# TrevorS/voxtral-mini-realtime-rs

Hardware: AMD Instinct MI355X
Metric: decode_tok_per_s (higher is better)
Workload: dtype f32

## Files before the change

voxtral-mini-realtime-rs_amd/csrc/vox_kernels.hip:

```cpp
#include "vox_kernels.h"

#include <hip/hip_fp16.h>

#include <unistd.h>

#include <algorithm>
#include <atomic>
#include <cstdio>
#include <cstdlib>
#include <cstring>
#include <string>
#include <mutex>
#include <unordered_map>

namespace vox {

static int g_tl_next = -1, g_tl_slots = 0;
#ifdef VOX_TIMELINE
__device__ unsigned long long* g_tl_buf = nullptr;
__device__ int g_tl_waves = 0;
__device__ __forceinline__ void tl_stamp(int slot, int wave_global, int k) {
    if (slot >= 0 && (wave_global & 3) == 0 && (threadIdx.x & 63) == 0 && g_tl_buf && wave_global < g_tl_waves)
        g_tl_buf[((size_t)slot * g_tl_waves + wave_global) * 4 + k] = wall_clock64();
}
// ... 483 lines not shown
    const int P = passes_for(p.w.K, R);
#define VOX_RP(R_, P_) if (R == R_ && P == P_) return gemv_dispatch_pe<P_, R_>(p, ny, pro, epi, s)
    VOX_RP(1, 1); VOX_RP(1, 2); VOX_RP(1, 3); VOX_RP(1, 5);
    VOX_RP(2, 1); VOX_RP(2, 2); VOX_RP(2, 3); VOX_RP(2, 4); VOX_RP(2, 5); VOX_RP(2, 9);
    VOX_RP(4, 1); VOX_RP(4, 2); VOX_RP(4, 6);
#undef VOX_RP
    return hipErrorInvalidValue;
}

const char* q4_gemv_kernel_name(int K, int pro, int epi, int R) {
    static thread_local char buf[96];
    snprintf(buf, sizeof buf, "q4_gemv_kernel<P=%d,R=%d,PRO=%d,EPI=%d,NWV=%d>", passes_for(K, R), R, pro, epi, gemv_fat_shape(K, R) ? q4_gemv_nwv(K, epi) : 4);
    return buf;
}

__device__ __forceinline__ float dot8_bf16(const uint4 w, const float4 xa, const float4 xb) {
    float s0 = __uint_as_float(w.x << 16) * xa.x, s1 = __uint_as_float(w.x & 0xFFFF0000u) * xa.y;
    s0 = fmaf(__uint_as_float(w.y << 16), xa.z, s0); s1 = fmaf(__uint_as_float(w.y & 0xFFFF0000u), xa.w, s1);
    s0 = fmaf(__uint_as_float(w.z << 16), xb.x, s0); s1 = fmaf(__uint_as_float(w.z & 0xFFFF0000u), xb.y, s1);
    s0 = fmaf(__uint_as_float(w.w << 16), xb.z, s0); s1 = fmaf(__uint_as_float(w.w & 0xFFFF0000u), xb.w, s1);
    return s0 + s1;
}

__device__ __forceinline__ float dot8_f32(const uint4 we, const uint4 wo, const float4 xa, const float4 xb) {
    float s0 = __uint_as_float(we.x) * xa.x, s1 = __uint_as_float(we.y) * xa.y;
    s0 = fmaf(__uint_as_float(we.z), xa.z, s0); s1 = fmaf(__uint_as_float(we.w), xa.w, s1);
    s0 = fmaf(__uint_as_float(wo.x), xb.x, s0); s1 = fmaf(__uint_as_float(wo.y), xb.y, s1);
    s0 = fmaf(__uint_as_float(wo.z), xb.z, s0); s1 = fmaf(__uint_as_float(wo.w), xb.w, s1);
    return s0 + s1;
}
template <int PRO, int EPI, int F32W = 0>
__global__ __launch_bounds__(256) VOX_NO_PK_F32 void dense_gemv_kernel(const GemvParams p) {
    constexpr int NX = 10, R = 2;
    extern __shared__ __attribute__((aligned(16))) float smem[];
    const int K = p.w.K, N = p.w.N, nc = K >> 3;
    float4* xe = reinterpret_cast<float4*>(smem);
    float4* xo = xe + nc;
    float* red = smem + K;
    const int tid = threadIdx.x, lane = tid & 63, wave = tid >> 6, y = blockIdx.y;
    const float* __restrict__ xg = p.x + (size_t)y * p.x_stride;
    const int npieces = K >> 2;
    float4 xp[NX];
    float ss = 0.f;
#pragma unroll
    for (int i = 0; i < NX; i++) {
        const int pc = tid + 256 * i;
        xp[i] = reinterpret_cast<const float4*>(xg)[min(pc, npieces - 1)];
        if (PRO != PRO_NONE && pc < npieces) ss += (xp[i].x * xp[i].x + xp[i].y * xp[i].y) + (xp[i].z * xp[i].z + xp[i].w * xp[i].w);
    }
    float rms = 1.0f;
    if (PRO != PRO_NONE) {
        ss = wave_sum(ss);
        if (lane == 0) red[wave] = ss;
        __syncthreads();
        rms = 1.0f / sqrtf(((red[0] + red[1]) + (red[2] + red[3])) / (float)K + p.eps);
    }
#pragma unroll
    for (int i = 0; i < NX; i++) {
        const int pc = tid + 256 * i;
        if (pc < npieces) {
            float4 v = xp[i];
            if (PRO != PRO_NONE) {
                const float4 gm = reinterpret_cast<const float4*>(p.gamma)[pc];
                v.x = (v.x * rms) * gm.x; v.y = (v.y * rms) * gm.y; v.z = (v.z * rms) * gm.z; v.w = (v.w * rms) * gm.w;
                if (PRO == PRO_RMS_MUL) {
                    const float4 m = reinterpret_cast<const float4*>(p.mul)[pc];
                    v.x *= m.x; v.y *= m.y; v.z *= m.z; v.w *= m.w;
                }
            }
            if (pc & 1) xo[pc >> 1] = v; else xe[pc >> 1] = v;
        }
    }
    __syncthreads();
    int best_i = 0x7fffffff; float best = -INFINITY;
    const int pos = (EPI == EPI_ROPE_KV) ? (p.pos_ptr ? *p.pos_ptr : 0) + p.pos_off : 0;
    const int n_groups = N / R, n_waves = gridDim.x * 4;
    for (int g = blockIdx.x * 4 + wave; g < n_groups; g += n_waves) {
        const int row0 = g * R;
        const uint4* w0 = (F32W ? p.w.qt : p.w.qs) + (size_t)row0 * nc * (F32W ? 2 : 1);
        const uint4* w1 = w0 + nc * (F32W ? 2 : 1);
        float acc[R] = {0.f, 0.f};
        for (int c0 = 0; c0 < nc; c0 += 128) {
            const int ca = c0 + lane, cb = ca + 64, cca = min(ca, nc - 1), ccb = min(cb, nc - 1);
            const float4 xea = xe[cca], xoa = xo[cca], xeb = xe[ccb], xob = xo[ccb];
            const float ma = ca < nc ? 1.0f : 0.0f, mb = cb < nc ? 1.0f : 0.0f;
            if (F32W) {
                const uint4 a0e = ld_nt_u4(w0 + 2 * cca), a0o = ld_nt_u4(w0 + 2 * cca + 1), a1e = ld_nt_u4(w0 + 2 * ccb), a1o = ld_nt_u4(w0 + 2 * ccb + 1);
                const uint4 b0e = ld_nt_u4(w1 + 2 * cca), b0o = ld_nt_u4(w1 + 2 * cca + 1), b1e = ld_nt_u4(w1 + 2 * ccb), b1o = ld_nt_u4(w1 + 2 * ccb + 1);
                acc[0] += ma * dot8_f32(a0e, a0o, xea, xoa) + mb * dot8_f32(a1e, a1o, xeb, xob);
                acc[1] += ma * dot8_f32(b0e, b0o, xea, xoa) + mb * dot8_f32(b1e, b1o, xeb, xob);
            } else {
                const uint4 a0 = ld_nt_u4(w0 + cca), a1 = ld_nt_u4(w0 + ccb), b0 = ld_nt_u4(w1 + cca), b1 = ld_nt_u4(w1 + ccb);
                acc[0] += ma * dot8_bf16(a0, xea, xoa) + mb * dot8_bf16(a1, xeb, xob);
                acc[1] += ma * dot8_bf16(b0, xea, xoa) + mb * dot8_bf16(b1, xeb, xob);
            }
        }
        acc[0] = wave_sum(acc[0]); acc[1] = wave_sum(acc[1]);
        if (EPI == EPI_STORE || EPI == EPI_RESID || EPI == EPI_GELU) {
#pragma unroll
            for (int r = 0; r < R; r++) {
                const int n = row0 + r;
                if (lane == r) {
                    float v = acc[r];
                    if (p.bias) v += p.bias[n];
                    if (EPI == EPI_RESID) v = v + p.resid[(size_t)y * p.resid_stride + n];
                    if (EPI == EPI_GELU) v = gelu_f(v);
                    p.out[(size_t)y * p.out_stride + n] = v;
                }
            }
        } else if (EPI == EPI_SWIGLU) {
            if (lane == 0) p.out[(size_t)y * p.out_stride + (row0 >> 1)] = silu_f(acc[0]) * acc[1];
        } else if (EPI == EPI_ROPE_KV) {
            const int hd = p.hd, half = hd >> 1, n = row0;
            if (lane == 0) {
                const float a = acc[0], b = acc[1];
                if (n < p.n_q + p.n_k) {
                    const int dd = n % hd;
                    const float c = p.rope_cos[(size_t)pos * half + (dd >> 1)], sn = p.rope_sin[(size_t)pos * half + (dd >> 1)];
                    const float ra = a * c - b * sn, rb = a * sn + b * c;
                    if (n < p.n_q) { p.out[n] = ra; p.out[n + 1] = rb; }
                    else {
                        const int kn = n - p.n_q, kh = kn / hd;
                        float* dst = p.kcache + (size_t)kh * p.cache_head_stride + (size_t)pos * hd + dd;
                        dst[0] = ra; dst[1] = rb;
                    }
                } else {
                    const int vn = n - p.n_q - p.n_k, vh = vn / hd, dd = vn % hd;
                    float* dst = p.vcache + (size_t)vh * p.cache_head_stride + (size_t)pos * hd + dd;
                    dst[0] = a; dst[1] = b;
                }
            }
        } else if (EPI == EPI_ARGMAX) {
#pragma unroll
            for (int r = 0; r < R; r++) {
                const int n = row0 + r;
                if (p.out && lane == r) p.out[(size_t)y * p.out_stride + n] = acc[r];
                argmax_take(best, best_i, acc[r], n);
            }
        }
    }
    if (EPI == EPI_ARGMAX) {
        if (lane == 0) { red[4 + wave] = best; reinterpret_cast<int*>(red)[8 + wave] = best_i; }
        __syncthreads();
        if (tid == 0) {
            float bv = red[4]; int bidx = reinterpret_cast<int*>(red)[8];
            for (int wv = 1; wv < 4; wv++) argmax_take(bv, bidx, red[4 + wv], reinterpret_cast<int*>(red)[8 + wv]);
            p.part_val[(size_t)y * gridDim.x + blockIdx.x] = bv;
            p.part_idx[(size_t)y * gridDim.x + blockIdx.x] = bidx;
        }
    }
}

int dense_gemv_grid(int N) { const int wgs = (N / 2 + 3) / 4; return wgs > 2048 ? 2048 : (wgs < 1 ? 1 : wgs); }

template <int PRO, int EPI>
static hipError_t dense_launch_t(const GemvParams& p, int ny, hipStream_t s) {
    const size_t lds = (size_t)(p.w.K + 16) * sizeof(float);
    gemm_form_note(GEMM_FORM_DENSE_GEMV);
    if (p.w.fmt == WFMT_F32) dense_gemv_kernel<PRO, EPI, 1><<<dim3(dense_gemv_grid(p.w.N), ny), dim3(256), lds, s>>>(p);
    else dense_gemv_kernel<PRO, EPI, 0><<<dim3(dense_gemv_grid(p.w.N), ny), dim3(256), lds, s>>>(p);
    return hipGetLastError();
}
static hipError_t launch_dense_gemv(const GemvParams& p, int ny, int pro, int epi, hipStream_t s) {
    if (p.w.K % 32 || p.w.K > 10240 || p.w.N % 2) return hipErrorInvalidValue;
    if ((pro == PRO_RMS_MUL || pro == PRO_RMS_MUL_SUM) && p.mul == nullptr) return hipErrorInvalidValue;
    if (pro == PRO_RMS_MUL_SUM) return hipErrorInvalidValue;
#define VOX_CASE(P_, E_) if (pro == P_ && epi == E_) return dense_launch_t<P_, E_>(p, ny, s)
    VOX_CASE(PRO_NONE, EPI_STORE); VOX_CASE(PRO_NONE, EPI_RESID); VOX_CASE(PRO_NONE, EPI_GELU); VOX_CASE(PRO_NONE, EPI_SWIGLU);
    VOX_CASE(PRO_RMS, EPI_STORE); VOX_CASE(PRO_RMS, EPI_ARGMAX); VOX_CASE(PRO_RMS, EPI_SWIGLU); VOX_CASE(PRO_RMS_MUL, EPI_SWIGLU);
    VOX_CASE(PRO_RMS, EPI_ROPE_KV);
#undef VOX_CASE
    return hipErrorInvalidValue;
}

typedef __attribute__((__vector_size__(8 * sizeof(__bf16)))) __bf16 bf16x8;
typedef __attribute__((__vector_size__(4 * sizeof(float)))) float f32x4;

__device__ __forceinline__ uint32_t bf16_rne_bits(float x) {
    const uint32_t u = __float_as_uint(x);
    return (u + 0x7FFFu + ((u >> 16) & 1u)) >> 16;
}
typedef __bf16 bf16x2_t __attribute__((ext_vector_type(2)));
typedef float f32x2_t __attribute__((ext_vector_type(2)));
__device__ __forceinline__ uint32_t cvt_pk_bf16(float a, float b) {
    const f32x2_t v = {a, b};
    union { bf16x2_t b; uint32_t u; } c; c.b = __builtin_convertvector(v, bf16x2_t); return c.u;
}
__device__ __forceinline__ void split_pair(float a, float b, uint32_t& hi, uint32_t& lo) {
    hi = cvt_pk_bf16(a, b);
    lo = cvt_pk_bf16(a - __uint_as_float(hi << 16), b - __uint_as_float(hi & 0xFFFF0000u));
}
__device__ __forceinline__ void split_bf16x8(const float4 a, const float4 b, uint4& hi, uint4& lo) {
    split_pair(a.x, a.y, hi.x, lo.x); split_pair(a.z, a.w, hi.y, lo.y);
    split_pair(b.x, b.y, hi.z, lo.z); split_pair(b.z, b.w, hi.w, lo.w);
}
__device__ __forceinline__ uint32_t pack_bf16_exact(float a, float b) {
    return (__float_as_uint(a) >> 16) | (__float_as_uint(b) & 0xFFFF0000u);
}
__device__ __forceinline__ uint4 q4_dword_to_bf16x8(uint32_t w) {
    const uint32_t lo = w & 0x0F0F0F0Fu, hi = (w >> 4) & 0x0F0F0F0Fu;
    uint4 o;
    o.x = pack_bf16_exact(ub0(lo) - 8.0f, ub1(lo) - 8.0f);
    o.y = pack_bf16_exact(ub2(lo) - 8.0f, ub3(lo) - 8.0f);
    o.z = pack_bf16_exact(ub0(hi) - 8.0f, ub1(hi) - 8.0f);
    o.w = pack_bf16_exact(ub2(hi) - 8.0f, ub3(hi) - 8.0f);
    return o;
}
__device__ __forceinline__ bf16x8 as_bf16x8(uint4 v) {
    union { uint4 u; bf16x8 b; } c; c.u = v; return c.b;
}

__device__ __forceinline__ uint4 q4_dword_to_bf16x8_biased(uint32_t w) {
    const uint32_t lo = w & 0x0F0F0F0Fu, hi = (w >> 4) & 0x0F0F0F0Fu, c = 0x43434343u;
    return make_uint4(__builtin_amdgcn_perm(lo, c, 0x00060004u), __builtin_amdgcn_perm(hi, c, 0x00060004u),
                      __builtin_amdgcn_perm(lo, c, 0x00070005u), __builtin_amdgcn_perm(hi, c, 0x00070005u));
}

__device__ __forceinline__ void xf_store4(uint16_t* __restrict__ xf, int K, int row, int k, float4 v) {
    const int q = k >> 7, j = (k >> 5) & 3, e = k & 31, half = e >> 4, g = (e & 15) >> 2;
    const size_t base = ((size_t)((q * 4 + j) * 64 + g * 16 + row)) * 8 + 2 * half;
    const size_t plane = (size_t)(K >> 7) * 256 * 8;
    uint32_t hi, lo;
    split_pair(v.x, v.z, hi, lo); *reinterpret_cast<uint32_t*>(xf + base) = hi; *reinterpret_cast<uint32_t*>(xf + plane + base) = lo;
    split_pair(v.y, v.w, hi, lo); *reinterpret_cast<uint32_t*>(xf + base + 4) = hi; *reinterpret_cast<uint32_t*>(xf + plane + base + 4) = lo;
}

template <int EPI, int FMT>
__global__ __launch_bounds__(256) __attribute__((amdgpu_waves_per_eu(2))) void q4_gemm_k32_kernel(const GemmParams p) {
    __shared__ __attribute__((aligned(16))) uint4 lds[2][2][256];
    const int K = p.w.K, nb = p.w.nb, N = p.w.N, M = p.M;
    (void)K;
    const int tid = threadIdx.x, lane = tid & 63, wave = tid >> 6;
    const int m0 = blockIdx.y * 64, n0 = blockIdx.x * 64;
    const int sm = tid >> 2, sg = tid & 3;
    const bool srow_ok = (m0 + sm) < M;
    const float* xrow = p.x + (size_t)(srow_ok ? (m0 + sm) : 0) * p.x_stride;
    const int slot = ((sm >> 4) * 4 + sg) * 16 + (sm & 15);
    const int wn = n0 + wave * 16 + (lane & 15), wg = lane >> 4;
    const bool wrow_ok = wn < N;
    const uint32_t* wq = reinterpret_cast<const uint32_t*>(p.w.qs) + (size_t)(wrow_ok ? wn : 0) * nb * 4 + wg;
    const uint16_t* ws = FMT == WFMT_Q4_0 ? p.w.sc + (size_t)(wrow_ok ? wn : 0) * nb : nullptr;
    const uint4* wd16 = p.w.qs + (size_t)(wrow_ok ? wn : 0) * nb * 4 + wg;
    const int xoff_a = FMT == WFMT_Q4_0 ? 4 * sg : 8 * sg, xoff_b = FMT == WFMT_Q4_0 ? 16 + 4 * sg : 8 * sg + 4;

    f32x4 acc[4];
#pragma unroll
    for (int i = 0; i < 4; i++) acc[i] = (f32x4){0.f, 0.f, 0.f, 0.f};

#define VOX_GLOAD(B_)                                                                              \
    xa = *reinterpret_cast<const float4*>(xrow + 32 * (B_) + xoff_a);        \
    xb = *reinterpret_cast<const float4*>(xrow + 32 * (B_) + xoff_b);                                               \
    if (FMT == WFMT_Q4_0) { wd = wq[(size_t)(B_) * 4]; wsc = ws[(B_)]; }    \
    else { wdv = wd16[(size_t)(B_) * 4]; }
#define VOX_STAGE(BUF_)                                                                            \
    { uint4 hi_, lo_; split_bf16x8(xa, xb, hi_, lo_); lds[(BUF_)][0][slot] = hi_; lds[(BUF_)][1][slot] = lo_; }
    float4 xa, xb; uint32_t wd = 0; uint16_t wsc = 0; uint4 wdv = make_uint4(0, 0, 0, 0);
    VOX_GLOAD(0)
    VOX_STAGE(0)
    uint32_t cur_wd = wd; uint16_t cur_sc = wsc; uint4 cur_wdv = wdv;
    { const int b1 = min(1, nb - 1); VOX_GLOAD(b1) }
    __syncthreads();
    for (int b = 0; b < nb; b++) {
        const int buf = b & 1;
        const float4 sxa = xa, sxb = xb; const uint32_t swd = wd; const uint16_t ssc = wsc; const uint4 swdv = wdv;
        { const int b2 = min(b + 2, nb - 1); VOX_GLOAD(b2) }
        const bf16x8 bw = as_bf16x8(FMT == WFMT_Q4_0 ? q4_dword_to_bf16x8(cur_wd) : cur_wdv);
        const float d = FMT == WFMT_Q4_0 ? f16_bits_to_f32(cur_sc) : 1.0f;
#pragma unroll
        for (int mt = 0; mt < 4; mt++) {
            const bf16x8 ah = as_bf16x8(lds[buf][0][mt * 64 + lane]);
            const bf16x8 al = as_bf16x8(lds[buf][1][mt * 64 + lane]);
            f32x4 t = __builtin_amdgcn_mfma_f32_16x16x32_bf16(ah, bw, (f32x4){0.f, 0.f, 0.f, 0.f}, 0, 0, 0);
            t = __builtin_amdgcn_mfma_f32_16x16x32_bf16(al, bw, t, 0, 0, 0);
            acc[mt][0] = fmaf(d, t[0], acc[mt][0]); acc[mt][1] = fmaf(d, t[1], acc[mt][1]);
            acc[mt][2] = fmaf(d, t[2], acc[mt][2]); acc[mt][3] = fmaf(d, t[3], acc[mt][3]);
        }
        if (b + 1 < nb) {
            uint4 hi_, lo_; split_bf16x8(sxa, sxb, hi_, lo_); lds[buf ^ 1][0][slot] = hi_; lds[buf ^ 1][1][slot] = lo_;
            cur_wd = swd; cur_sc = ssc; cur_wdv = swdv;
        }
        __syncthreads();
    }
#undef VOX_GLOAD
#undef VOX_STAGE
    const float bias = (p.bias && wrow_ok) ? p.bias[wn] : 0.f;
#pragma unroll
    for (int mt = 0; mt < 4; mt++)
#pragma unroll
        for (int r = 0; r < 4; r++) {
            const int m = m0 + mt * 16 + 4 * (lane >> 4) + r;
            float v = acc[mt][r] + bias;
            if (EPI == EPI_SWIGLU) {
                const float other = dpp_mov<0xB1>(v);
                if (m < M && wrow_ok && !(wn & 1)) p.out[(size_t)m * p.out_stride + (wn >> 1)] = silu_f(v) * other;
            } else if (m < M && wrow_ok) {
                if (EPI == EPI_RESID) v = v + p.resid[(size_t)m * p.resid_stride + wn];
                if (EPI == EPI_GELU) v = gelu_f(v);
                p.out[(size_t)m * p.out_stride + wn] = v;
            }
        }
}

template <int MT, int NT, int EPI, int FMT, int TB = 0>
__global__ __launch_bounds__(256) __attribute__((amdgpu_waves_per_eu(2))) void q4_gemm_kernel(const GemmParams p) {
    extern __shared__ __attribute__((aligned(16))) uint4 glds[];
    constexpr int PLANE = 4 * MT * 64, BUF = 2 * PLANE;
    const int nb = p.w.nb, N = p.w.N, M = p.M, nq = nb >> 2;
    const int tid = threadIdx.x, lane = tid & 63, wave = tid >> 6;
    const int m0 = blockIdx.y * (16 * MT), n0 = blockIdx.x * (64 * NT);
    const int KSP = p.ksplit > 1 ? p.ksplit : 1, kz = blockIdx.z;
    const int qb = (int)((long)nq * kz / KSP), qe = (int)((long)nq * (kz + 1) / KSP);
    const float* xrow[MT]; int slot[MT], xo_a[MT], xo_b[MT];
#pragma unroll
    for (int i = 0; i < MT; i++) {
        const int f = tid + 256 * i, sm = f >> 4, j = (f >> 2) & 3, g = f & 3;
        xrow[i] = p.x + (size_t)min(m0 + sm, M - 1) * p.x_stride;
        slot[i] = (j * MT + (sm >> 4)) * 64 + g * 16 + ((sm & 15) ^ (4 * j + g));
        xo_a[i] = 32 * j + (FMT == WFMT_Q4_0 ? 4 * g : 8 * g); xo_b[i] = 32 * j + (FMT == WFMT_Q4_0 ? 16 + 4 * g : 8 * g + 4);
    }
    const int wg = lane >> 4;
    int rdl[4];
#pragma unroll
    for (int j = 0; j < 4; j++) rdl[j] = (lane & 48) | ((lane & 15) ^ (4 * j + wg));
    const uint32_t* wq[NT]; const uint16_t* ws[NT]; const uint4* wd16[NT]; const uint4* wqt[NT]; int wn[NT]; bool wok[NT];
#pragma unroll
    for (int t = 0; t < NT; t++) {
        wn[t] = n0 + (wave * NT + t) * 16 + (lane & 15); wok[t] = wn[t] < N;
        const size_t row = (size_t)min(wn[t], N - 1);
        wq[t] = reinterpret_cast<const uint32_t*>(p.w.qs) + row * nb * 4 + wg;
        ws[t] = FMT == WFMT_Q4_0 ? p.w.sc + row * nb : nullptr;
        wd16[t] = p.w.qs + row * nb * 4 + wg;
        const size_t T = (size_t)min((n0 >> 4) + wave * NT + t, ((N + 15) >> 4) - 1);
        wqt[t] = TB ? p.w.qt + T * nq * 64 + lane : nullptr;
    }
    f32x4 acc[NT][MT];
#pragma unroll
    for (int t = 0; t < NT; t++)
#pragma unroll
        for (int i = 0; i < MT; i++) acc[t][i] = (f32x4){0.f, 0.f, 0.f, 0.f};

    float4 xa[MT], xb[MT];
    uint32_t wd[NT][4]; uint2 wsc[NT]; uint4 wdv[NT][4];
#define VOX_GLOAD(Q_)                                                                                          \
    _Pragma("unroll") for (int i = 0; i < MT; i++) {                                                           \
        xa[i] = *reinterpret_cast<const float4*>(xrow[i] + 128 * (Q_) + xo_a[i]);                              \
        xb[i] = *reinterpret_cast<const float4*>(xrow[i] + 128 * (Q_) + xo_b[i]);                              \
    }                                                                                                          \
    _Pragma("unroll") for (int t = 0; t < NT; t++) {                                                           \
        if (FMT == WFMT_Q4_0) {                                                                                \
            if (TB) { const uint4 w4 = ld_nt_u4(wqt[t] + (size_t)64 * (Q_)); wd[t][0] = w4.x; wd[t][1] = w4.y; wd[t][2] = w4.z; wd[t][3] = w4.w; } \
            else { _Pragma("unroll") for (int j = 0; j < 4; j++) wd[t][j] = wq[t][(size_t)(4 * (Q_) + j) * 4]; } \
            wsc[t] = *reinterpret_cast<const uint2*>(ws[t] + 4 * (Q_));                                        \
        } else {                                                                                               \
            _Pragma("unroll") for (int j = 0; j < 4; j++) wdv[t][j] = wd16[t][(size_t)(4 * (Q_) + j) * 4];     \
        }                                                                                                      \
    }
#define VOX_STAGE(BUF_)                                                                                        \
    _Pragma("unroll") for (int i = 0; i < MT; i++) {                                                           \
        uint4 hi_, lo_; split_bf16x8(sxa[i], sxb[i], hi_, lo_);                                                \
        glds[(BUF_) * BUF + slot[i]] = hi_; glds[(BUF_) * BUF + PLANE + slot[i]] = lo_;                        \
    }
    VOX_GLOAD(qb)
    float4 sxa[MT], sxb[MT];
#pragma unroll
    for (int i = 0; i < MT; i++) { sxa[i] = xa[i]; sxb[i] = xb[i]; }
    VOX_STAGE(0)
    uint32_t cwd[NT][4]; uint2 csc[NT]; uint4 cwdv[NT][4];
#pragma unroll
    for (int t = 0; t < NT; t++) { csc[t] = wsc[t];
#pragma unroll
        for (int j = 0; j < 4; j++) { cwd[t][j] = wd[t][j]; cwdv[t][j] = wdv[t][j]; } }
    { const int q1 = min(qb + 1, qe - 1); VOX_GLOAD(q1) }
    __syncthreads();
    for (int q = qb; q < qe; q++) {
        const int buf = (q - qb) & 1;
#pragma unroll
        for (int i = 0; i < MT; i++) { sxa[i] = xa[i]; sxb[i] = xb[i]; }
        uint32_t nwd[NT][4]; uint2 nsc[NT]; uint4 nwdv[NT][4];
#pragma unroll
        for (int t = 0; t < NT; t++) { nsc[t] = wsc[t];
#pragma unroll
            for (int j = 0; j < 4; j++) { nwd[t][j] = wd[t][j]; nwdv[t][j] = wdv[t][j]; } }
        { const int q2 = min(q + 2, qe - 1); VOX_GLOAD(q2) }
#pragma unroll
        for (int j = 0; j < 4; j++) {
#pragma unroll
            for (int t = 0; t < NT; t++) {
                const bf16x8 bw = as_bf16x8(FMT == WFMT_Q4_0 ? q4_dword_to_bf16x8(cwd[t][j]) : cwdv[t][j]);
                float d = 1.0f;
                if (FMT == WFMT_Q4_0) {
                    const uint32_t pr = (j & 2) ? csc[t].y : csc[t].x;
                    d = f16_bits_to_f32((uint16_t)((j & 1) ? (pr >> 16) : (pr & 0xFFFFu)));
                }
#pragma unroll
                for (int i = 0; i < MT; i++) {
                    const bf16x8 ah = as_bf16x8(glds[buf * BUF + (j * MT + i) * 64 + rdl[j]]);
                    const bf16x8 al = as_bf16x8(glds[buf * BUF + PLANE + (j * MT + i) * 64 + rdl[j]]);
                    f32x4 tt = __builtin_amdgcn_mfma_f32_16x16x32_bf16(ah, bw, (f32x4){0.f, 0.f, 0.f, 0.f}, 0, 0, 0);
                    tt = __builtin_amdgcn_mfma_f32_16x16x32_bf16(al, bw, tt, 0, 0, 0);
                    acc[t][i][0] = fmaf(d, tt[0], acc[t][i][0]); acc[t][i][1] = fmaf(d, tt[1], acc[t][i][1]);
                    acc[t][i][2] = fmaf(d, tt[2], acc[t][i][2]); acc[t][i][3] = fmaf(d, tt[3], acc[t][i][3]);
                }
            }
        }
        if (q + 1 < qe) {
            VOX_STAGE(buf ^ 1)
#pragma unroll
            for (int t = 0; t < NT; t++) { csc[t] = nsc[t];
#pragma unroll
                for (int j = 0; j < 4; j++) { cwd[t][j] = nwd[t][j]; cwdv[t][j] = nwdv[t][j]; } }
        }
        __syncthreads();
    }
#undef VOX_GLOAD
#undef VOX_STAGE
#pragma unroll
    for (int t = 0; t < NT; t++) {
        const float bias = (p.bias && wok[t] && kz == 0) ? p.bias[wn[t]] : 0.f;
#pragma unroll
        for (int i = 0; i < MT; i++)
#pragma unroll
            for (int r = 0; r < 4; r++) {
                const int m = m0 + i * 16 + 4 * (lane >> 4) + r;
                float v = acc[t][i][r] + bias;
                if (EPI == EPI_SWIGLU) {
                    const float other = dpp_mov<0xB1>(v);
                    if (m < M && wok[t] && !(wn[t] & 1)) p.out[(size_t)m * p.out_stride + (wn[t] >> 1)] = silu_f(v) * other;
                } else if (m < M && wok[t]) {
                    if (EPI == EPI_RESID) v = v + p.resid[(size_t)m * p.resid_stride + wn[t]];
                    if (EPI == EPI_GELU) v = gelu_f(v);
                    (p.out + (size_t)kz * p.M * p.out_stride)[(size_t)m * p.out_stride + wn[t]] = v;
                }
            }
    }
}

__global__ void q4_tile_build_kernel(Q4W w, uint4* __restrict__ qt, uint16_t* __restrict__ st, int n_tiles) {
    const int nq = w.nb >> 2;
    const long total = (long)n_tiles * nq * 64;
    for (long i = (long)blockIdx.x * blockDim.x + threadIdx.x; i < total; i += (long)gridDim.x * blockDim.x) {
        const int lane = (int)(i & 63); const long tq = i >> 6; const int q = (int)(tq % nq), T = (int)(tq / nq);
        const int g = lane >> 4, n = T * 16 + (lane & 15);
        uint32_t d[4] = {0x88888888u, 0x88888888u, 0x88888888u, 0x88888888u};
        if (n < w.N) {
            const uint32_t* src = reinterpret_cast<const uint32_t*>(w.qs) + ((size_t)n * w.nb + 4 * q) * 4 + g;
#pragma unroll
            for (int j = 0; j < 4; j++) d[j] = src[j * 4];
        }
        qt[i] = make_uint4(d[0], d[1], d[2], d[3]);
        if (g == 0) {
#pragma unroll
            for (int j = 0; j < 4; j++) st[(tq * 16 + (lane & 15)) * 4 + j] = n < w.N ? w.sc[(size_t)n * w.nb + 4 * q + j] : (uint16_t)0;
        }
    }
}
hipError_t launch_q4_tile_build(Q4W w, uint4* qt, uint16_t* st, hipStream_t s) {
    if (w.nb % 4) return hipErrorInvalidValue;
    const int n_tiles = (w.N + 15) / 16;
    q4_tile_build_kernel<<<dim3(2048), dim3(256), 0, s>>>(w, qt, st, n_tiles);
    return hipGetLastError();
}

template <int NTW, int EPI, int TILED, int XIN, int PRO, int STEPS = 0>
__global__ __launch_bounds__(NTW == 3 ? 256 : 512, NTW == 3 ? 3 : 1) void q4_skinny_kernel(const GemmParams p) {
    extern __shared__ __attribute__((aligned(16))) float sred[];
    __shared__ float s_rstd[16]; __shared__ float s_pp[32 * 16];
    constexpr bool KVP = EPI == EPI_ROPE_KV_PAGED, ROPE_KV = EPI == EPI_ROPE_KV || KVP;
    const int nb = p.w.nb, N = p.w.N, M = p.M, nq = nb >> 2;
    const int tid = threadIdx.x, lane = tid & 63, wave = tid >> 6, KS = blockDim.x >> 6;
    const int g = lane >> 4, li = lane & 15;
    const int nbase = blockIdx.x * (16 * NTW);
    const int tlw = wave == 0 ? (int)blockIdx.x * 4 : 1; (void)tlw;
    VOX_TL(p.tl_slot, tlw, 0);
    const float* xrow = p.x + (size_t)min(li, M - 1) * p.x_stride;
    const uint4* wq[NTW]; const uint16_t* ws[NTW];
    const int n_tiles = (N + 15) >> 4;
#pragma unroll
    for (int t = 0; t < NTW; t++) {
        if (TILED) {
            const size_t T = (size_t)min(blockIdx.x * NTW + t, n_tiles - 1);
            wq[t] = p.w.qt + T * nq * 64 + lane; ws[t] = p.w.st + (T * nq * 16 + li) * 4;
        } else {
            const size_t row = (size_t)min(nbase + t * 16 + li, N - 1);
            wq[t] = p.w.qs + row * nb + g; ws[t] = p.w.sc + row * nb;
        }
    }
    f32x4 acc[NTW];
#pragma unroll
    for (int t = 0; t < NTW; t++) acc[t] = (f32x4){0.f, 0.f, 0.f, 0.f};
    uint4 wv[NTW], wvn[NTW]; uint2 sv[NTW], svn[NTW]; float4 xa[4], xb[4];
    const uint4* xfh = p.xf + lane; const uint4* xfl = p.xf + (size_t)nq * 256 + lane;
#define VOX_WLOAD(WV_, SV_, Q_)                                                                            \
    _Pragma("unroll") for (int t = 0; t < NTW; t++) {                                                      \
        WV_[t] = ld_nt_u4(wq[t] + (TILED ? 64 : 4) * (Q_)); SV_[t] = *reinterpret_cast<const uint2*>(ws[t] + (TILED ? 64 : 4) * (Q_)); }
#define VOX_XLOAD(Q_)                                                                                      \
    _Pragma("unroll") for (int j = 0; j < 4; j++) {                                                        \
        if (XIN) {                                                                                         \
            xa[j] = *reinterpret_cast<const float4*>(xfh + ((Q_) * 4 + j) * 64);                           \
            xb[j] = *reinterpret_cast<const float4*>(xfl + ((Q_) * 4 + j) * 64);                           \
        } else {                                                                                           \
            xa[j] = *reinterpret_cast<const float4*>(xrow + 128 * (Q_) + 32 * j + 4 * g);                  \
            xb[j] = *reinterpret_cast<const float4*>(xrow + 128 * (Q_) + 32 * j + 16 + 4 * g); } }
#define VOX_SSTEP(WV_, SV_, XA_, XB_)                                                                      \
    {                                                                                                      \
        const bf16x8 m136 = as_bf16x8(make_uint4(0xC308C308u, 0xC308C308u, 0xC308C308u, 0xC308C308u));     \
        uint32_t dw[NTW][4];                                                                               \
        _Pragma("unroll") for (int t = 0; t < NTW; t++) {                                                  \
            dw[t][0] = WV_[t].x; dw[t][1] = WV_[t].y; dw[t][2] = WV_[t].z; dw[t][3] = WV_[t].w;            \
            if (!TILED) {                            \
                auto s01 = __builtin_amdgcn_permlane16_swap(WV_[t].x, WV_[t].y, false, false);             \
                auto s23 = __builtin_amdgcn_permlane16_swap(WV_[t].z, WV_[t].w, false, false);             \
                auto u02 = __builtin_amdgcn_permlane32_swap(s01[0], s23[0], false, false);                 \
                auto u13 = __builtin_amdgcn_permlane32_swap(s01[1], s23[1], false, false);                 \
                dw[t][0] = u02[0]; dw[t][1] = u13[0]; dw[t][2] = u02[1]; dw[t][3] = u13[1];                \
            }                                                                                              \
        }                                                                                                  \
               \
        _Pragma("unroll") for (int j = 0; j < 4; j++) {                                                    \
            uint4 ah, al;                                                                                  \
            if (XIN) {                                                                                     \
                ah = make_uint4(__float_as_uint(XA_[j].x), __float_as_uint(XA_[j].y), __float_as_uint(XA_[j].z), __float_as_uint(XA_[j].w)); \
                al = make_uint4(__float_as_uint(XB_[j].x), __float_as_uint(XB_[j].y), __float_as_uint(XB_[j].z), __float_as_uint(XB_[j].w)); \
            } else {                                                                                       \
                split_pair(XA_[j].x, XA_[j].z, ah.x, al.x); split_pair(XB_[j].x, XB_[j].z, ah.y, al.y);    \
                split_pair(XA_[j].y, XA_[j].w, ah.z, al.z); split_pair(XB_[j].y, XB_[j].w, ah.w, al.w);    \
            }                                                                                              \
            const f32x4 sx = __builtin_amdgcn_mfma_f32_16x16x32_bf16(as_bf16x8(ah), m136, (f32x4){0.f, 0.f, 0.f, 0.f}, 0, 0, 0); \
            const f32x4 cs = __builtin_amdgcn_mfma_f32_16x16x32_bf16(as_bf16x8(al), m136, sx, 0, 0, 0);    \
            _Pragma("unroll") for (int t = 0; t < NTW; t++) {                                              \
                const bf16x8 bw = as_bf16x8(q4_dword_to_bf16x8_biased(dw[t][j]));                          \
                const uint32_t sc2 = (j >> 1) ? SV_[t].y : SV_[t].x;                                       \
                const float d = f16_bits_to_f32((uint16_t)((j & 1) ? (sc2 >> 16) : (sc2 & 0xFFFFu)));      \
                f32x4 tt = __builtin_amdgcn_mfma_f32_16x16x32_bf16(as_bf16x8(ah), bw, cs, 0, 0, 0);        \
                tt = __builtin_amdgcn_mfma_f32_16x16x32_bf16(as_bf16x8(al), bw, tt, 0, 0, 0);              \
                acc[t] = __builtin_elementwise_fma((f32x4){d, d, d, d}, tt, acc[t]);                        \
            }                                                                                              \
        }                                                                                                  \
    }
    float pv[12]; const int prow = tid & 15, pch = tid >> 4, nch = blockDim.x >> 4;
    float pre_res[4] = {0.f, 0.f, 0.f, 0.f}; float pre_xw = 0.f; int pre_pos[4] = {0, 0, 0, 0}; int pre_row[4] = {0, 0, 0, 0}; int pre_kvp[4] = {0, 0, 0, 0};
#define VOX_PRELOADS                                                                                       \
    {                                                                                                      \
        if (PRO) {                                                                                         \
            _Pragma("unroll") for (int u = 0; u < 12; u++) {                                               \
                const int pi = pch + u * nch;                                                              \
                const float v = p.ssq_part[(size_t)min(pi, p.n_part - 1) * 16 + prow];                     \
                pv[u] = pi < p.n_part ? v : 0.f;                                                           \
            }                                                                                              \
        }                                                                                                  \
        const int n0_ = min(nbase + min(wave, NTW - 1) * 16 + li, N - 1);                                  \
        if (EPI == EPI_RESID_XF || EPI == EPI_RESID) {                                                     \
            _Pragma("unroll") for (int r = 0; r < 4; r++) pre_res[r] = p.resid[(size_t)min(4 * g + r, M - 1) * p.resid_stride + n0_]; \
        }                                                                                                  \
        if (EPI == EPI_RESID_XF) { pre_xw = p.xf_w[n0_]; if (p.xf_w2) pre_xw *= p.xf_w2[n0_]; }            \
        if (ROPE_KV) {                                                                                     \
            _Pragma("unroll") for (int r = 0; r < 4; r++) pre_pos[r] = p.pos[min(4 * g + r, M - 1)];       \
            _Pragma("unroll") for (int r = 0; r < 4; r++) pre_row[r] = p.kv_row ? p.kv_row[min(4 * g + r, M - 1)] : min(4 * g + r, M - 1); \
            if (KVP) { _Pragma("unroll") for (int r = 0; r < 4; r++) pre_kvp[r] = p.kv_pos[min(4 * g + r, M - 1)]; } \
        }                                                                                                  \
    }
    constexpr bool STRAIGHT = STEPS > 0 && TILED && XIN;
    if (!STRAIGHT) VOX_PRELOADS
    const int per = (nq + KS - 1) / KS;
    int q = TILED ? wave * per : wave;
    const int qend = TILED ? min(q + per, nq) : nq, qs = TILED ? 1 : KS;
    if (STRAIGHT) {
        constexpr int D = NTW >= 3 ? 2 : 3, DB = STEPS <= 0 ? 1 : (D < STEPS ? D : STEPS);
        uint4 wr[DB][NTW]; uint2 sr[DB][NTW]; float4 xr[DB][2][4];
#define VOX_ISSUE(B_, Q_)                                                                                  \
        { VOX_WLOAD(wr[B_], sr[B_], (Q_))                                                                  \
          _Pragma("unroll") for (int j = 0; j < 4; j++) {                                                  \
              xr[B_][0][j] = *reinterpret_cast<const float4*>(xfh + ((Q_) * 4 + j) * 64);                  \
              xr[B_][1][j] = *reinterpret_cast<const float4*>(xfl + ((Q_) * 4 + j) * 64); } }
        VOX_ISSUE(0, q)
        __builtin_amdgcn_sched_barrier(0);
        VOX_PRELOADS
        __builtin_amdgcn_sched_barrier(0);
#pragma unroll
        for (int u = 1; u < DB; u++) VOX_ISSUE(u, q + u)
#pragma unroll
        for (int st = 0; st < STEPS; st++) {
            __builtin_amdgcn_sched_barrier(0);
            VOX_SSTEP(wr[st % DB], sr[st % DB], xr[st % DB][0], xr[st % DB][1])
            if (st == 0 && PRO) s_pp[pch * 16 + prow] = ((pv[0] + pv[1]) + (pv[2] + pv[3])) + ((pv[4] + pv[5]) + (pv[6] + pv[7])) + ((pv[8] + pv[9]) + (pv[10] + pv[11]));
            if (st + DB < STEPS) VOX_ISSUE(st % DB, q + st + DB)
            if (st == 0) { VOX_TL(p.tl_slot, tlw, 1); }
        }
#undef VOX_ISSUE
    } else if (q < qend) {
        VOX_WLOAD(wv, sv, q)
        for (;;) {
            { const int qn = min(q + qs, qend - 1); VOX_WLOAD(wvn, svn, qn) }
            VOX_XLOAD(q)
            __builtin_amdgcn_sched_barrier(0);
            VOX_SSTEP(wv, sv, xa, xb)
            VOX_TL(p.tl_slot, tlw, 1);
            q += qs; if (q >= qend) break;
            { const int qn = min(q + qs, qend - 1); VOX_WLOAD(wv, sv, qn) }
            VOX_XLOAD(q)
            __builtin_amdgcn_sched_barrier(0);
            VOX_SSTEP(wvn, svn, xa, xb)
            q += qs; if (q >= qend) break;
        }
    }
#undef VOX_WLOAD
#undef VOX_XLOAD
#undef VOX_SSTEP
#undef VOX_PRELOADS
    VOX_TL(p.tl_slot, tlw, 2);
#pragma unroll
    for (int t = 0; t < NTW; t++)
        *reinterpret_cast<float4*>(sred + ((size_t)(wave * NTW + t) * 64 + lane) * 4) = make_float4(acc[t][0], acc[t][1], acc[t][2], acc[t][3]);
    if (PRO && !STRAIGHT) s_pp[pch * 16 + prow] = ((pv[0] + pv[1]) + (pv[2] + pv[3])) + ((pv[4] + pv[5]) + (pv[6] + pv[7])) + ((pv[8] + pv[9]) + (pv[10] + pv[11]));
    __syncthreads();
    if (PRO) {
        if (tid < 16) { float a = 0.f; for (int cch = 0; cch < nch; cch++) a += s_pp[cch * 16 + tid]; s_rstd[tid] = 1.0f / sqrtf(a / (float)p.w.K + p.norm_eps); }
        __syncthreads();
    }
    for (int t = wave; t < NTW; t += KS) {
        float4 sum = make_float4(0.f, 0.f, 0.f, 0.f);
        for (int w = 0; w < KS; w++) {
            const float4 v = *reinterpret_cast<const float4*>(sred + ((size_t)(w * NTW + t) * 64 + lane) * 4);
            sum.x += v.x; sum.y += v.y; sum.z += v.z; sum.w += v.w;
        }
        if (PRO) { const float4 rs = *reinterpret_cast<const float4*>(s_rstd + 4 * g); sum.x *= rs.x; sum.y *= rs.y; sum.z *= rs.z; sum.w *= rs.w; }
        const int n = nbase + t * 16 + li; const bool nok = n < N;
        const float bias = (p.bias && nok) ? p.bias[n] : 0.f;
        const float vals[4] = {sum.x + bias, sum.y + bias, sum.z + bias, sum.w + bias};
        float xw = 0.f;
        const bool pre = t == wave;
        if (EPI == EPI_RESID_XF && nok) { if (pre) xw = pre_xw; else { xw = p.xf_w[n]; if (p.xf_w2) xw *= p.xf_w2[n]; } }
#pragma unroll
        for (int r = 0; r < 4; r++) {
            const int m = 4 * g + r;
            float v = vals[r];
            if (EPI == EPI_SWIGLU) {
                const float other = dpp_mov<0xB1>(v);
                if (m < M && nok && !(n & 1)) p.out[(size_t)m * p.out_stride + (n >> 1)] = silu_f(v) * other;
            } else if (EPI == EPI_SWIGLU_XF) {
                const float a = silu_f(v) * dpp_mov<0xB1>(v);
                const float b = __shfl(a, lane + 4, 64);
                const int k = n >> 1;
                if (m < M && nok && !(n & 1) && !(k & 2)) {
                    uint32_t hi, lo; split_pair(a, b, hi, lo);
                    const int K2 = N >> 1, qq = k >> 7, jj = (k >> 5) & 3, e = k & 31, half = e >> 4, gg = (e & 15) >> 2, tt = e & 3;
                    const size_t base = ((size_t)((qq * 4 + jj) * 64 + gg * 16 + m)) * 8 + 2 * half + 4 * (tt & 1);
                    uint16_t* xo = reinterpret_cast<uint16_t*>(p.out);
                    *reinterpret_cast<uint32_t*>(xo + base) = hi; *reinterpret_cast<uint32_t*>(xo + (size_t)(K2 >> 7) * 256 * 8 + base) = lo;
                }
            } else if (EPI == EPI_RESID_XF) {
                const bool ok = m < M && nok;
                if (ok) { v = v + (pre ? pre_res[r] : p.resid[(size_t)m * p.resid_stride + n]); p.out[(size_t)m * p.out_stride + n] = v; } else v = 0.f;
                const float ss = row16_sum(v * v);
                if (li == 0) p.ssq_out[(size_t)blockIdx.x * 16 + m] = ss;
                const float a = v * xw, b = dpp_mov<0x4E>(a);
                if (ok && !(li & 2)) {
                    uint32_t hi, lo; split_pair(a, b, hi, lo);
                    const int qq = n >> 7, jj = (n >> 5) & 3, e = n & 31, half = e >> 4, gg = (e & 15) >> 2, tt = e & 3;
                    const size_t base = ((size_t)((qq * 4 + jj) * 64 + gg * 16 + m)) * 8 + 2 * half + 4 * (tt & 1);
                    *reinterpret_cast<uint32_t*>(p.xf_out + base) = hi; *reinterpret_cast<uint32_t*>(p.xf_out + (size_t)(N >> 7) * 256 * 8 + base) = lo;
                }
            } else if (ROPE_KV) {
                const float other = dpp_mov<0xB1>(v);
                if (m < M && nok) {
                    const int ps = pre ? pre_pos[r] : p.pos[m], kd = p.n_kv * p.hd;
                    const int cr = pre ? pre_row[r] : (p.kv_row ? p.kv_row[m] : m);
                    const int cp = KVP ? (pre ? pre_kvp[r] : p.kv_pos[m]) : ps;
                    if (n < p.n_q + kd) {
                        const int dd = n % p.hd;
                        const size_t ti = (size_t)ps * (p.hd >> 1) + (dd >> 1);
                        const float c = p.rope_cos[ti], sn = p.rope_sin[ti];
                        const float o = (n & 1) ? other * sn + v * c : v * c - other * sn;
                        if (n < p.n_q) p.out[(size_t)m * p.out_stride + n] = o;
                        else p.kc[(size_t)cr * p.kv_seq_stride + (size_t)((n - p.n_q) / p.hd) * p.kv_head_stride + (size_t)cp * p.hd + dd] = o;
                    } else {
                        const int vn = n - p.n_q - kd;
                        p.vc[(size_t)cr * p.kv_seq_stride + (size_t)(vn / p.hd) * p.kv_head_stride + (size_t)cp * p.hd + (vn % p.hd)] = v;
                    }
                }
            } else if (m < M && nok) {
                if (EPI == EPI_RESID) v = v + (pre ? pre_res[r] : p.resid[(size_t)m * p.resid_stride + n]);
                if (EPI == EPI_GELU) v = gelu_f(v);
                p.out[(size_t)m * p.out_stride + n] = v;
            }
        }
    }
    VOX_TL(p.tl_slot, tlw, 3);
}

typedef unsigned int u32x2_t __attribute__((ext_vector_type(2)));
__device__ __forceinline__ bf16x8 v4_as_bf16x8(u32x4_t v) { union { u32x4_t u; bf16x8 b; } c; c.u = v; return c.b; }
template <int MT, int NTW, bool DIRECT>
__global__ __launch_bounds__(256, 2) void q4_wide_kernel(const GemmParams p, const int sps, float* __restrict__ planes) {
    extern __shared__ __attribute__((aligned(16))) u32x4_t wlds[];
    __shared__ float s_rstd[MT * 16]; __shared__ float s_pp[16 * 16];
    __shared__ __attribute__((aligned(16))) float s_cs[2][MT][4][4][4];
    constexpr int STAGE = MT * 8 * 64, NA = 2 * MT;
    const int N = p.w.N, nq = p.w.nb >> 2, n_tiles = (N + 15) >> 4;
    const int tid = threadIdx.x, lane = tid & 63, wave = tid >> 6, g = lane >> 4, li = lane & 15;
    const int tile0 = ((int)blockIdx.x * 4 + wave) * NTW, q0 = (int)blockIdx.y * sps;
    const uint4* wq[NTW]; const uint16_t* ws[NTW];
#pragma unroll
    for (int t = 0; t < NTW; t++) {
        const size_t T = (size_t)min(tile0 + t, n_tiles - 1);
        wq[t] = p.w.qt + (T * nq + q0) * 64 + lane; ws[t] = p.w.st + ((T * nq + q0) * 16 + li) * 4;
    }
    const u32x4_t* asrc[NA];
#pragma unroll
    for (int u = 0; u < NA; u++) {
        const int i = tid + 256 * u, line = i >> 6, mt = line >> 3, hl = (line >> 2) & 1, j = line & 3;
        asrc[u] = reinterpret_cast<const u32x4_t*>(p.xf) + (size_t)mt * p.xf_gstride + (size_t)hl * nq * 256 + ((size_t)q0 * 4 + j) * 64 + (i & 63);
    }
    f32x4 acc[MT][NTW];
#pragma unroll
    for (int mt = 0; mt < MT; mt++)
#pragma unroll
// ... 3242 lines not shown
```

Baseline: 1495.

## Use shallower prefetch pipeline and higher occupancy for 2x2 Q4 transposed GEMM

```diff
diff --git a/voxtral-mini-realtime-rs_amd/csrc/vox_kernels.hip b/voxtral-mini-realtime-rs_amd/csrc/vox_kernels.hip
--- a/voxtral-mini-realtime-rs_amd/csrc/vox_kernels.hip
+++ b/voxtral-mini-realtime-rs_amd/csrc/vox_kernels.hip
@@ -809,7 +809,7 @@
 }
 
 template <int MT, int NT, int EPI, int FMT, int TB = 0>
-__global__ __launch_bounds__(256) __attribute__((amdgpu_waves_per_eu(2))) void q4_gemm_kernel(const GemmParams p) {
+__global__ __launch_bounds__(256) __attribute__((amdgpu_waves_per_eu(MT == 2 && NT == 2 && FMT == WFMT_Q4_0 && TB == 1 ? 3 : 2))) void q4_gemm_kernel(const GemmParams p) {
     extern __shared__ __attribute__((aligned(16))) uint4 glds[];
     constexpr int PLANE = 4 * MT * 64, BUF = 2 * PLANE;
     const int nb = p.w.nb, N = p.w.N, M = p.M, nq = nb >> 2;
@@ -867,58 +867,86 @@
         uint4 hi_, lo_; split_bf16x8(sxa[i], sxb[i], hi_, lo_);                                                \
         glds[(BUF_) * BUF + slot[i]] = hi_; glds[(BUF_) * BUF + PLANE + slot[i]] = lo_;                        \
     }
-    VOX_GLOAD(qb)
+#define VOX_MMA                                                                                                \
+        _Pragma("unroll") for (int j = 0; j < 4; j++) {                                                                \
+            _Pragma("unroll") for (int t = 0; t < NT; t++) {                                                           \
+                const bf16x8 bw = as_bf16x8(FMT == WFMT_Q4_0 ? q4_dword_to_bf16x8(cwd[t][j]) : cwdv[t][j]);            \
+                float d = 1.0f;                                                                                        \
+                if (FMT == WFMT_Q4_0) {                                                                                \
+                    const uint32_t pr = (j & 2) ? csc[t].y : csc[t].x;                                                 \
+                    d = f16_bits_to_f32((uint16_t)((j & 1) ? (pr >> 16) : (pr & 0xFFFFu)));                            \
+                }                                                                                                      \
+                _Pragma("unroll") for (int i = 0; i < MT; i++) {                                                       \
+                    const bf16x8 ah = as_bf16x8(glds[buf * BUF + (j * MT + i) * 64 + rdl[j]]);                         \
+                    const bf16x8 al = as_bf16x8(glds[buf * BUF + PLANE + (j * MT + i) * 64 + rdl[j]]);                 \
+                    f32x4 tt = __builtin_amdgcn_mfma_f32_16x16x32_bf16(ah, bw, (f32x4){0.f, 0.f, 0.f, 0.f}, 0, 0, 0);  \
+                    tt = __builtin_amdgcn_mfma_f32_16x16x32_bf16(al, bw, tt, 0, 0, 0);                                 \
+                    acc[t][i][0] = fmaf(d, tt[0], acc[t][i][0]); acc[t][i][1] = fmaf(d, tt[1], acc[t][i][1]);          \
+                    acc[t][i][2] = fmaf(d, tt[2], acc[t][i][2]); acc[t][i][3] = fmaf(d, tt[3], acc[t][i][3]);          \
+                }                                                                                                      \
+            }                                                                                                          \
+        }
     float4 sxa[MT], sxb[MT];
-#pragma unroll
-    for (int i = 0; i < MT; i++) { sxa[i] = xa[i]; sxb[i] = xb[i]; }
-    VOX_STAGE(0)
     uint32_t cwd[NT][4]; uint2 csc[NT]; uint4 cwdv[NT][4];
-#pragma unroll
-    for (int t = 0; t < NT; t++) { csc[t] = wsc[t];
-#pragma unroll
-        for (int j = 0; j < 4; j++) { cwd[t][j] = wd[t][j]; cwdv[t][j] = wdv[t][j]; } }
-    { const int q1 = min(qb + 1, qe - 1); VOX_GLOAD(q1) }
-    __syncthreads();
-    for (int q = qb; q < qe; q++) {
-        const int buf = (q - qb) & 1;
+    if constexpr (MT == 2 && NT == 2 && FMT == WFMT_Q4_0 && TB == 1) {
+        VOX_GLOAD(qb)
 #pragma unroll
         for (int i = 0; i < MT; i++) { sxa[i] = xa[i]; sxb[i] = xb[i]; }
-        uint32_t nwd[NT][4]; uint2 nsc[NT]; uint4 nwdv[NT][4];
-#pragma unroll
-        for (int t = 0; t < NT; t++) { nsc[t] = wsc[t];
-#pragma unroll
-            for (int j = 0; j < 4; j++) { nwd[t][j] = wd[t][j]; nwdv[t][j] = wdv[t][j]; } }
-        { const int q2 = min(q + 2, qe - 1); VOX_GLOAD(q2) }
-#pragma unroll
-        for (int j = 0; j < 4; j++) {
-#pragma unroll
-            for (int t = 0; t < NT; t++) {
-                const bf16x8 bw = as_bf16x8(FMT == WFMT_Q4_0 ? q4_dword_to_bf16x8(cwd[t][j]) : cwdv[t][j]);
-                float d = 1.0f;
-                if (FMT == WFMT_Q4_0) {
-                    const uint32_t pr = (j & 2) ? csc[t].y : csc[t].x;
-                    d = f16_bits_to_f32((uint16_t)((j & 1) ? (pr >> 16) : (pr & 0xFFFFu)));
-                }
-#pragma unroll
-                for (int i = 0; i < MT; i++) {
-                    const bf16x8 ah = as_bf16x8(glds[buf * BUF + (j * MT + i) * 64 + rdl[j]]);
-                    const bf16x8 al = as_bf16x8(glds[buf * BUF + PLANE + (j * MT + i) * 64 + rdl[j]]);
-                    f32x4 tt = __builtin_amdgcn_mfma_f32_16x16x32_bf16(ah, bw, (f32x4){0.f, 0.f, 0.f, 0.f}, 0, 0, 0);
-                    tt = __builtin_amdgcn_mfma_f32_16x16x32_bf16(al, bw, tt, 0, 0, 0);
-                    acc[t][i][0] = fmaf(d, tt[0], acc[t][i][0]); acc[t][i][1] = fmaf(d, tt[1], acc[t][i][1]);
-                    acc[t][i][2] = fmaf(d, tt[2], acc[t][i][2]); acc[t][i][3] = fmaf(d, tt[3], acc[t][i][3]);
-                }
+        VOX_STAGE(0)
+#pragma unroll
+        for (int t = 0; t < NT; t++) { csc[t] = wsc[t];
+#pragma unroll
+            for (int j = 0; j < 4; j++) cwd[t][j] = wd[t][j]; }
+        __syncthreads();
+        for (int q = qb; q < qe; q++) {
+            const int buf = (q - qb) & 1;
+            { const int q1 = min(q + 1, qe - 1); VOX_GLOAD(q1) }
+            __builtin_amdgcn_sched_barrier(0);
+            VOX_MMA
+            if (q + 1 < qe) {
+#pragma unroll
+                for (int i = 0; i < MT; i++) { sxa[i] = xa[i]; sxb[i] = xb[i]; }
+                VOX_STAGE(buf ^ 1)
+#pragma unroll
+                for (int t = 0; t < NT; t++) { csc[t] = wsc[t];
+#pragma unroll
+                    for (int j = 0; j < 4; j++) cwd[t][j] = wd[t][j]; }
             }
-        }
-        if (q + 1 < qe) {
-            VOX_STAGE(buf ^ 1)
-#pragma unroll
-            for (int t = 0; t < NT; t++) { csc[t] = nsc[t];
-#pragma unroll
-                for (int j = 0; j < 4; j++) { cwd[t][j] = nwd[t][j]; cwdv[t][j] = nwdv[t][j]; } }
-        }
+            __syncthreads();
+        }
+    } else {
+        VOX_GLOAD(qb)
+#pragma unroll
+        for (int i = 0; i < MT; i++) { sxa[i] = xa[i]; sxb[i] = xb[i]; }
+        VOX_STAGE(0)
+#pragma unroll
+        for (int t = 0; t < NT; t++) { csc[t] = wsc[t];
+#pragma unroll
+            for (int j = 0; j < 4; j++) { cwd[t][j] = wd[t][j]; cwdv[t][j] = wdv[t][j]; } }
+        { const int q1 = min(qb + 1, qe - 1); VOX_GLOAD(q1) }
         __syncthreads();
-    }
+        for (int q = qb; q < qe; q++) {
+            const int buf = (q - qb) & 1;
+#pragma unroll
+            for (int i = 0; i < MT; i++) { sxa[i] = xa[i]; sxb[i] = xb[i]; }
+            uint32_t nwd[NT][4]; uint2 nsc[NT]; uint4 nwdv[NT][4];
+#pragma unroll
+            for (int t = 0; t < NT; t++) { nsc[t] = wsc[t];
+#pragma unroll
+                for (int j = 0; j < 4; j++) { nwd[t][j] = wd[t][j]; nwdv[t][j] = wdv[t][j]; } }
+            { const int q2 = min(q + 2, qe - 1); VOX_GLOAD(q2) }
+            VOX_MMA
+            if (q + 1 < qe) {
+                VOX_STAGE(buf ^ 1)
+#pragma unroll
+                for (int t = 0; t < NT; t++) { csc[t] = nsc[t];
+#pragma unroll
+                    for (int j = 0; j < 4; j++) { cwd[t][j] = nwd[t][j]; cwdv[t][j] = nwdv[t][j]; } }
+            }
+            __syncthreads();
+        }
+    }
+#undef VOX_MMA
 #undef VOX_GLOAD
 #undef VOX_STAGE
 #pragma unroll
```

Result: faster. 1510, median of 6 (+1.0%).
